# DavidSlayback/po-brax

Measured on AMD Instinct MI355X. Metric: env-steps/sec AntHeavenHell batch 65536 @1/2/4/8 GPU; % HBM roofline, higher is better.
Workload: dtype f32; 1 GPU; ant_heavenhell B=65536/GPU (global 65536), create(batch_size=B) autoreset chain, episode_length 1000, PBD 10 substeps, random uniform(-1,1) actions (threefry); env=ant_heavenhell, global_batch=65536, batch_per_gpu=65536, episode_length=1000, qp_storage=f32, parallelism=env-shard x1 (strong: global batch split), dynamics=pbd, obs_mask=none, obs_mask_columns=0, launch=hipGraph replay of the K steps

## Files before the change

po-brax_amd/csrc/pob_blockwalk.h:

```cpp
#pragma once
#include <stdint.h>
#ifdef POB_BW_HOST
#define POB_BW_D static inline
#else
#define POB_BW_D __device__ __forceinline__
#endif

#define QBW_WAVES 4
#define QBW_WCAP 50
#define QBW_SLOT_DW 11
#define QBW_CON_DW 5
#define QBW_LANE_MAX 64
#define QBW_CAP (QBW_WAVES * QBW_WCAP)
#define QBW_SEG_FLOATS (QBW_WCAP * QBW_SLOT_DW + 1)
#define QBW_NO_CONTACT (-1)

POB_BW_D constexpr int bw_item_off(const int j) { return QBW_SLOT_DW * j; }
POB_BW_D constexpr int bw_meta_off(const int j) { return QBW_SLOT_DW * j + 2 * QBW_CON_DW; }
POB_BW_D constexpr int bw_con_off(const int c) { return QBW_SLOT_DW * (c >> 1) + QBW_CON_DW * (c & 1); }
POB_BW_D constexpr int bw_count_off() { return QBW_WCAP * QBW_SLOT_DW; }

POB_BW_D constexpr int bw_meta(const int bit, const bool seg, const int slot) { return bit | (seg ? 64 : 0) | (slot << 7); }
POB_BW_D constexpr int bw_meta_bit(const int m) { return m & 63; }
POB_BW_D constexpr bool bw_meta_seg(const int m) { return (m & 64) != 0; }
POB_BW_D constexpr int bw_meta_slot(const int m) { return (m >> 7) & 3; }

POB_BW_D int bw_lane_count(const uint64_t m0, const uint64_t m1, const uint64_t m2) {
  const int n = __builtin_popcountll(m0) + __builtin_popcountll(m1) + __builtin_popcountll(m2);
  return n < QBW_LANE_MAX ? n : QBW_LANE_MAX;
}
POB_BW_D void bw_prefix_step(const uint64_t m, const int lane, const int b, int &base, int &tot) {
  base += __builtin_popcountll(m & ((1ull << lane) - 1ull)) << b;
  tot += __builtin_popcountll(m) << b;
}
#define QBW_PREFIX_BITS 7

POB_BW_D bool bw_next_item(uint64_t (&M)[3], int &slot, int &bit) {
  const bool h0 = M[0] != 0ull, h1 = M[1] != 0ull, h2 = M[2] != 0ull;
  const bool has = h0 | h1 | h2;
  slot = h0 ? 0 : (h1 ? 1 : 2);
  const uint64_t ml = h0 ? M[0] : (h1 ? M[1] : M[2]);
  bit = has ? __builtin_ctzll(ml) : 0;
  const uint64_t pop = has ? ml & (0ull - ml) : 0ull;
  M[0] = h0 ? M[0] & ~pop : M[0];
  M[1] = (!h0 & h1) ? M[1] & ~pop : M[1];
  M[2] = (!h0 & !h1) ? M[2] & ~pop : M[2];
  return has;
}

struct BwDeal {
  int off[QBW_WAVES];
  int T;
  bool ovf;
};
POB_BW_D BwDeal bw_deal(const int n0, const int n1, const int n2, const int n3, const int cap) {
  BwDeal d;
  d.off[0] = 0; d.off[1] = n0; d.off[2] = n0 + n1; d.off[3] = n0 + n1 + n2;
  const int T = n0 + n1 + n2 + n3;
  d.ovf = (T > cap) | (n0 > QBW_WCAP) | (n1 > QBW_WCAP) | (n2 > QBW_WCAP) | (n3 > QBW_WCAP);
  d.T = d.ovf ? 0 : T;
  return d;
}
POB_BW_D int bw_rounds(const BwDeal &d) { return (d.T + 7) >> 3; }
POB_BW_D int bw_first_round(const int w, const int sub) { return (w + sub) & (QBW_WAVES - 1); }
POB_BW_D void bw_item_owner(const BwDeal &d, const int i, int &w, int &j) {
  w = (i >= d.off[1] ? 1 : 0) + (i >= d.off[2] ? 1 : 0) + (i >= d.off[3] ? 1 : 0);
  j = i - (w == 0 ? 0 : (w == 1 ? d.off[1] : (w == 2 ? d.off[2] : d.off[3])));
}
POB_BW_D void bw_apply_range(const int base, const int n, const bool ovf, int &c0, int &c1) {
  c0 = 2 * base;
  c1 = ovf ? c0 : 2 * (base + n);
}
POB_BW_D void bw_body_ranges(const int base, const int n0, const int n1, const int n2, const bool ovf, int (&c)[4]) {
  c[0] = 2 * base;
  c[1] = ovf ? c[0] : c[0] + 2 * n0;
  c[2] = ovf ? c[0] : c[1] + 2 * n1;
  c[3] = ovf ? c[0] : c[2] + 2 * n2;
}
```

po-brax_amd/csrc/pob_kernels.hip:

```cpp
#include <hip/hip_fp16.h>
#include <hip/hip_runtime.h>

#include <climits>
#include <cstdio>
#include <cstdlib>
#include <cstring>
#include <mutex>
#include <new>
#include <type_traits>
#include <vector>

#include "../../include/pob.h"

#ifndef POB_QUAD_PRIO
#define POB_QUAD_PRIO 1
#endif
#ifndef POB_OCT_PRIO
#define POB_OCT_PRIO 1
#endif
#ifndef POB_HEX_PRIO
#define POB_HEX_PRIO 1
#endif
#include "pob_quad.h"
#include "pob_octet.h"
#include "pob_hexa.h"
#include "pob_physics.h"

namespace pob {
void default_params(pob_params &p);
const char *build_system(int kind, const pob_params &p, pob_sys &s);
int gather_grid(const pob_params &p, float *xyz, int cap);
}

struct pob_env {
  pob_sys sys;
  pob_sys *d_sys = nullptr;
  pob_params params;
  float *d_grid = nullptr;
  uint32_t *d_scratch = nullptr;
  int device = 0;
  int n_cu = 256;
};

#define POB_MIXED (-1)
#define POB_F_STAGED (1u << 16)
#define POB_F_INT_FORCE_FIXUP (1u << 30)
#define POB_F_INT_BWCAP_SHIFT 20
#define POB_F_INT_BWCAP_MASK (0xFFu << POB_F_INT_BWCAP_SHIFT)
#define POB_F_INTERNAL (POB_F_STAGED | POB_F_INT_FORCE_FIXUP | POB_F_INT_BWCAP_MASK)
#define POB_F_PUBLIC (POB_F_EPISODE | POB_F_AUTORESET | POB_F_ZERO_STEPS_ON_DONE)

#define POB_STATE_FIELDS(X)                                                                    \
  X(pos) X(rot) X(vel) X(ang) X(obs) X(reward) X(done) X(steps) X(truncation) X(m0) X(m1) X(m2) \
  X(rng) X(first_pos) X(first_rot) X(first_vel) X(first_ang) X(first_obs) X(any_done) X(done_u8) X(trunc_i32) \
  X(m0_i32) X(m1_i32) X(any_done_clear) X(obs_masked) X(ovf_mark)

struct StatePtrs {
  float *pos, *rot, *vel, *ang, *obs, *reward, *done, *steps, *truncation, *m0, *m1, *m2;
  uint32_t *rng;
  float *first_pos, *first_rot, *first_vel, *first_ang, *first_obs;
  uint32_t *any_done;
  uint8_t *done_u8;
  int32_t *trunc_i32, *m0_i32, *m1_i32;
  uint32_t *any_done_clear;
  float *obs_masked;
  uint8_t *ovf_mark;
};
POB_D void store_obs_masked(csys_t &S, float *dst, const float *stg, const int rows, const int D, const int lane) {
  const int K = S.obs_mask_n;
  for (int r = 0; r < rows; ++r)
    for (int c = lane; c < K; c += 64) dst[(size_t)r * K + c] = stg[r * D + S.obs_mask[c]];
}
static StatePtrs to_ptrs(const pob_state &s) {
  StatePtrs p;
#define POB_CP(f) p.f = s.f;
  POB_STATE_FIELDS(POB_CP)
#undef POB_CP
  return p;
}

template <typename QT> struct Q;
template <> struct Q<float> {
  static POB_D float ld(const float *p, size_t i) { return p[i]; }
  static POB_D void st(float *p, size_t i, float v) { p[i] = v; }
};
template <> struct Q<__half> {
  static POB_D float ld(const float *p, size_t i) { return __half2float(reinterpret_cast<const __half *>(p)[i]); }
  static POB_D void st(float *p, size_t i, float v) {
    asm volatile("" : "+v"(v));
    reinterpret_cast<__half *>(p)[i] = __float2half_rn(v);
  }
};
template <typename QT> POB_D v3 ld3(const float *p, size_t i) {
  return V(Q<QT>::ld(p, i), Q<QT>::ld(p, i + 1), Q<QT>::ld(p, i + 2));
}
template <typename QT> POB_D void st3(float *p, size_t i, v3 v) {
  Q<QT>::st(p, i, v.x); Q<QT>::st(p, i + 1, v.y); Q<QT>::st(p, i + 2, v.z);
}
template <typename QT> POB_D q4 ld4(const float *p, size_t i) {
  q4 q; q.w = Q<QT>::ld(p, i); q.x = Q<QT>::ld(p, i + 1); q.y = Q<QT>::ld(p, i + 2); q.z = Q<QT>::ld(p, i + 3);
  return q;
}
// ... 677 lines not shown
#endif
    constexpr int KBIT = KIND < 0 ? 16 : 1 << KIND;
    constexpr bool FASTP = (POB_QUAD_FAST_PASS & KBIT) != 0, REDER = (POB_QUAD_REDERIVE & KBIT) != 0;
    if (LEG) {
#pragma nounroll
      for (int it = 0; it < Sp->substeps; ++it) qlegacy_substep<KIND != POB_ANT>(Sp, LT, WT, bd, a, Ls);
    } else {
#if defined(POB_EXP_NO_COLLIDE)
#pragma nounroll
    for (int it = 0; it < 2 * iters; ++it) qpbd_substep<KIND != POB_ANT>(Sp, LT, WT, bd, a, Ls, false, S.friction);
#elif defined(POB_EXP_NO_PHYSICS)
#pragma nounroll
    for (int it = 0; it < 0 * iters; ++it) qpbd_substep<KIND != POB_ANT>(Sp, LT, WT, bd, a, Ls, false, S.friction);
#else
    constexpr bool TWO = KIND == POB_GATHER && POB_QUAD_TWO_PASS;
    constexpr bool WALLS = KIND != POB_ANT;
    int pass = TWO ? (__any(qwall_mask_margin(S, bd, POB_QUAD_NEAR_MARGIN) != 0u) ? 1 : 0) : 1;
    auto reload = [&]() {
#pragma unroll
      for (int l = 0; l < QNB; ++l) {
        const int g = qbody_global(l, k);
        bd.x[l] = ld3<QT>(in.pos, r3 + 3 * g);
        bd.q[l] = ld4<QT>(in.rot, r4 + 4 * g);
        bd.v[l] = ld3<QT>(in.vel, r3 + 3 * g);
        bd.w[l] = ld3<QT>(in.ang, r3 + 3 * g);
        Ls.set3(l, QF_CV, V(0.0f, 0.0f, 0.0f));
        Ls.set3(l, QF_CA, V(0.0f, 0.0f, 0.0f));
      }
    };
    for (;;) {
    if (pass == 0) {
      bool near = false;
#pragma nounroll
      for (int it = 0; it < 2 * iters; ++it) {
#if POB_QUAD_PRIO == 1
        const int lvl = (it * 4) / (2 * iters);
        if (lvl == 0) __builtin_amdgcn_s_setprio(3);
        else if (lvl == 1) __builtin_amdgcn_s_setprio(2);
        else if (lvl == 2) __builtin_amdgcn_s_setprio(1);
        else __builtin_amdgcn_s_setprio(0);
#endif
        qpbd_substep<false, true>(Sp, LT, WT, bd, a, Ls, (it & 1) != 0, fric, &near);
      }
      if (!__any(near)) break;
      pass = 1;
      reload();
      continue;
    }
#ifndef POB_QUAD_SLOW_OOL
#define POB_QUAD_SLOW_OOL 1
#endif
    if constexpr (MODE == 1 && WALLS && COOP) {
      const int capf = (int)((flags & POB_F_INT_BWCAP_MASK) >> POB_F_INT_BWCAP_SHIFT);
      QBlock blk{lds + QPOOL_OFF, __builtin_amdgcn_readfirstlane((int)threadIdx.x >> 6), 0,
                 capf != 0 ? capf : QBW_CAP, dead, false};
#pragma nounroll
      for (int it = 0; it < 2 * iters; ++it) {
#if POB_QUAD_PRIO == 1
        const int lvl = (it * 4) / (2 * iters);
        if (lvl == 0) __builtin_amdgcn_s_setprio(3);
        else if (lvl == 1) __builtin_amdgcn_s_setprio(2);
        else if (lvl == 2) __builtin_amdgcn_s_setprio(1);
        else __builtin_amdgcn_s_setprio(0);
#endif
        qpbd_substep<WALLS, false, false, true>(Sp, LT, WT, bd, a, Ls, (it & 1) != 0, fric, nullptr, nullptr, &blk);
      }
      if (dead) return;
      if (blk.ovf || (flags & POB_F_INT_FORCE_FIXUP)) {
        if (lane == 0) out.ovf_mark[b_first] = 1;
        return;
      }
      break;
    }
    if (MODE == 1 && WALLS) {
      bool ovf = false;
#pragma nounroll
      for (int it = 0; it < 2 * iters; ++it) {
#if POB_QUAD_PRIO == 1
        const int lvl = (it * 4) / (2 * iters);
        if (lvl == 0) __builtin_amdgcn_s_setprio(3);
        else if (lvl == 1) __builtin_amdgcn_s_setprio(2);
        else if (lvl == 2) __builtin_amdgcn_s_setprio(1);
        else __builtin_amdgcn_s_setprio(0);
#endif
        qpbd_substep<WALLS, false, false>(Sp, LT, WT, bd, a, Ls, (it & 1) != 0, fric, nullptr, &ovf);
        if (__any(ovf)) break;
      }
      if (__any(ovf) || (flags & POB_F_INT_FORCE_FIXUP)) {
        if (lane == 0) out.ovf_mark[b_first] = 1;
        return;
      }
      break;
    }
    if (pass == 1 && WALLS && FASTP && MODE == 0) {
      bool ovf = false;
#pragma nounroll
      for (int it = 0; it < 2 * iters; ++it) {
#if POB_QUAD_PRIO == 1
        const int lvl = (it * 4) / (2 * iters);
        if (lvl == 0) __builtin_amdgcn_s_setprio(3);
        else if (lvl == 1) __builtin_amdgcn_s_setprio(2);
        else if (lvl == 2) __builtin_amdgcn_s_setprio(1);
        else __builtin_amdgcn_s_setprio(0);
#endif
        qpbd_substep<WALLS, false, false>(Sp, LT, WT, bd, a, Ls, (it & 1) != 0, fric, nullptr, &ovf);
        if (__any(ovf)) break;
      }
      if (!__any(ovf)) break;
// ... 1631 lines not shown
    }
  }
  switch (kind) {
    case POB_HEAVENHELL: hipLaunchKernelGGL((k_step_hex<POB_HEAVENHELL, QT, GACC>), g, b, 0, st, sp, B, pi, act, po, flags, L); break;
    case POB_GATHER: hipLaunchKernelGGL((k_step_hex<POB_GATHER, QT, GACC>), g, b, 0, st, sp, B, pi, act, po, flags, L); break;
    case POB_TAG: hipLaunchKernelGGL((k_step_hex<POB_TAG, QT, GACC>), g, b, 0, st, sp, B, pi, act, po, flags, L); break;
    default: hipLaunchKernelGGL((k_step_hex<POB_ANT, QT, GACC>), g, b, 0, st, sp, B, pi, act, po, flags, L); break;
  }
}
template <typename QT>
static void launch_step_hex(int kind, int n_cu, hipStream_t st, const void *sp, int B, const StatePtrs &pi,
                            const float *act, const StatePtrs &po, uint32_t flags, int L) {
  const char *f = getenv("POB_HEX_GACC");
  const bool acc = f ? atoi(f) != 0 : (kind == POB_HEAVENHELL || kind == POB_TAG || (B + 3) / 4 <= 4 * n_cu);
  if (acc) launch_step_hex_g<QT, true>(kind, st, sp, B, pi, act, po, flags, L, n_cu);
  else launch_step_hex_g<QT, false>(kind, st, sp, B, pi, act, po, flags, L, n_cu);
}
template <typename QT, bool GACC>
static void launch_step_oct_g(int kind, hipStream_t st, const void *sp, int B, const StatePtrs &pi, const float *act,
                              const StatePtrs &po, uint32_t flags, int L) {
  const dim3 g((unsigned)((B + 7) / 8)), b(64);
  switch (kind) {
    case POB_HEAVENHELL: hipLaunchKernelGGL((k_step_oct<POB_HEAVENHELL, QT, GACC>), g, b, 0, st, sp, B, pi, act, po, flags, L); break;
    case POB_GATHER: hipLaunchKernelGGL((k_step_oct<POB_GATHER, QT, GACC>), g, b, 0, st, sp, B, pi, act, po, flags, L); break;
    case POB_TAG: hipLaunchKernelGGL((k_step_oct<POB_TAG, QT, GACC>), g, b, 0, st, sp, B, pi, act, po, flags, L); break;
    default: hipLaunchKernelGGL((k_step_oct<POB_ANT, QT, GACC>), g, b, 0, st, sp, B, pi, act, po, flags, L); break;
  }
}
template <typename QT>
static void launch_step_oct(int kind, int n_cu, hipStream_t st, const void *sp, int B, const StatePtrs &pi,
                            const float *act, const StatePtrs &po, uint32_t flags, int L) {
  const char *f = getenv("POB_OCT_GACC");
  const bool acc = f ? atoi(f) != 0 : (B + 7) / 8 <= 4 * n_cu;
  if (acc) launch_step_oct_g<QT, true>(kind, st, sp, B, pi, act, po, flags, L);
  else launch_step_oct_g<QT, false>(kind, st, sp, B, pi, act, po, flags, L);
}
#ifndef POB_QUAD_SPLIT_KINDS
#define POB_QUAD_SPLIT_KINDS 23
#endif
static bool quad_split_launch(int kind) {
  const char *f = getenv("POB_QUAD_SPLIT");
  if (f) return atoi(f) != 0;
  return ((POB_QUAD_SPLIT_KINDS >> (kind < 0 ? 4 : kind)) & 1) != 0;
}
static uint32_t quad_force_fixup() {
  const char *f = getenv("POB_QUAD_FORCE_FIXUP");
  return f && atoi(f) != 0 ? POB_F_INT_FORCE_FIXUP : 0u;
}
static uint32_t quad_block_cap() {
  const char *f = getenv("POB_QUAD_BLOCK_CAP");
  const int n = f ? atoi(f) : 0;
  return n >= 1 && n < QBW_CAP ? (uint32_t)n << POB_F_INT_BWCAP_SHIFT : 0u;
}
template <typename QT>
static void launch_step_quad(int kind, bool legacy, int n_cu, hipStream_t st, const void *sp, int B,
                             const StatePtrs &pi, const float *act, const StatePtrs &po, uint32_t flags, int L) {
  const int bs = 4 * B <= 64 * 256 ? 64 : 256;
  const dim3 g = grid_for(4 * B, bs), b(bs);
  if (legacy) {
    switch (kind) {
      case POB_HEAVENHELL: hipLaunchKernelGGL((k_step_legacy<POB_HEAVENHELL, QT>), g, b, 0, st, sp, B, pi, act, po, flags, L); break;
      case POB_GATHER: hipLaunchKernelGGL((k_step_legacy<POB_GATHER, QT>), g, b, 0, st, sp, B, pi, act, po, flags, L); break;
      case POB_TAG: hipLaunchKernelGGL((k_step_legacy<POB_TAG, QT>), g, b, 0, st, sp, B, pi, act, po, flags, L); break;
      default: hipLaunchKernelGGL((k_step_legacy<POB_ANT, QT>), g, b, 0, st, sp, B, pi, act, po, flags, L); break;
    }
    return;
  }
  if (kind == POB_GATHER && (size_t)4 * B <= (size_t)3 * 64 * 4 * n_cu) {
    hipLaunchKernelGGL((k_step_quad_ga3<QT>), g, b, 0, st, sp, B, pi, act, po, flags, L);
    return;
  }
  const bool split = quad_split_launch(kind) && po.ovf_mark != nullptr;
  flags |= split ? quad_force_fixup() : 0u;
  const bool coop = split && bs == 256 && (kind == POB_HEAVENHELL || kind == POB_TAG);
  flags |= coop ? quad_block_cap() : 0u;
  switch (kind) {
    case POB_HEAVENHELL:
      if (split) {
        if (coop) hipLaunchKernelGGL((k_step_quad<POB_HEAVENHELL, QT, 1, true>), g, b, 0, st, sp, B, pi, act, po, flags, L);
        else hipLaunchKernelGGL((k_step_quad<POB_HEAVENHELL, QT, 1>), g, b, 0, st, sp, B, pi, act, po, flags, L);
        hipLaunchKernelGGL((k_step_quad<POB_HEAVENHELL, QT, 2>), g, b, 0, st, sp, B, pi, act, po, flags, L);
      } else {
        hipLaunchKernelGGL((k_step_quad<POB_HEAVENHELL, QT>), g, b, 0, st, sp, B, pi, act, po, flags, L);
      }
      break;
    case POB_GATHER:
      if (split) {
        hipLaunchKernelGGL((k_step_quad<POB_GATHER, QT, 1>), g, b, 0, st, sp, B, pi, act, po, flags, L);
        hipLaunchKernelGGL((k_step_quad<POB_GATHER, QT, 2>), g, b, 0, st, sp, B, pi, act, po, flags, L);
      } else {
        hipLaunchKernelGGL((k_step_quad<POB_GATHER, QT>), g, b, 0, st, sp, B, pi, act, po, flags, L);
      }
      break;
    case POB_TAG:
      if (split) {
        if (coop) hipLaunchKernelGGL((k_step_quad<POB_TAG, QT, 1, true>), g, b, 0, st, sp, B, pi, act, po, flags, L);
        else hipLaunchKernelGGL((k_step_quad<POB_TAG, QT, 1>), g, b, 0, st, sp, B, pi, act, po, flags, L);
        hipLaunchKernelGGL((k_step_quad<POB_TAG, QT, 2>), g, b, 0, st, sp, B, pi, act, po, flags, L);
      } else {
        hipLaunchKernelGGL((k_step_quad<POB_TAG, QT>), g, b, 0, st, sp, B, pi, act, po, flags, L);
      }
      break;
    default: hipLaunchKernelGGL((k_step_quad<POB_ANT, QT>), g, b, 0, st, sp, B, pi, act, po, flags, L); break;
  }
}
extern "C" {

int pob_abi_version(void) { return POB_ABI_VERSION; }
const char *pob_last_error(void) { return g_err; }

int pob_default_params(pob_params *p) {
  if (!p) return fail(POB_EINVAL, "params is NULL");
  pob::default_params(*p);
  return POB_OK;
}

static std::mutex g_grave_mu;
static std::vector<void *> g_grave;

static void drain_grave() {
  std::vector<void *> dead;
  {
    std::lock_guard<std::mutex> lk(g_grave_mu);
    dead.swap(g_grave);
  }
  for (void *p : dead) (void)hipFree(p);
}

// ... 295 lines not shown
```

po-brax_amd/csrc/pob_quad.h:

```cpp
#pragma once
#include "pob_physics.h"

#define QNB 3
#define QNJ 2

struct QBody {
  v3 x[QNB];
  q4 q[QNB];
  v3 v[QNB];
  v3 w[QNB];
};

template <int J>
POB_D float quad_bcast(float x) {
  float r;
  if (J == 0)
    asm volatile("s_nop 1\n\tv_mov_b32_dpp %0, %1 quad_perm:[0,0,0,0] row_mask:0xf bank_mask:0xf" : "=&v"(r) : "v"(x));
  else if (J == 1)
    asm volatile("s_nop 1\n\tv_mov_b32_dpp %0, %1 quad_perm:[1,1,1,1] row_mask:0xf bank_mask:0xf" : "=&v"(r) : "v"(x));
  else if (J == 2)
    asm volatile("s_nop 1\n\tv_mov_b32_dpp %0, %1 quad_perm:[2,2,2,2] row_mask:0xf bank_mask:0xf" : "=&v"(r) : "v"(x));
  else
    asm volatile("s_nop 1\n\tv_mov_b32_dpp %0, %1 quad_perm:[3,3,3,3] row_mask:0xf bank_mask:0xf" : "=&v"(r) : "v"(x));
  return r;
// ... 47 lines not shown
  }
  POB_D static constexpr int torso_off(int f) {
    return f == QF_PX ? QLT_PX : (f == QF_PQ ? QLT_PQ : (f == QF_CV ? QLT_CV : QLT_CA));
  }
  POB_D float *at(int l, int f, int i) const {
    return l == 0 ? base + 64 * QLL_FLOATS + 16 * (torso_off(f) + i) + (t >> 2) : base + 64 * (lane_off(l, f) + i) + t;
  }
  POB_D v3 get3(int l, int f) const { return V(*at(l, f, 0), *at(l, f, 1), *at(l, f, 2)); }
  POB_D q4 get4(int l, int f) const {
    q4 q; q.w = *at(l, f, 0); q.x = *at(l, f, 1); q.y = *at(l, f, 2); q.z = *at(l, f, 3); return q;
  }
  POB_D void set3(int l, int f, v3 v) const {
    if (l != 0 || (t & 3) == 0) { *at(l, f, 0) = v.x; *at(l, f, 1) = v.y; *at(l, f, 2) = v.z; }
  }
  POB_D void set4(int l, int f, q4 q) const {
    if (l != 0 || (t & 3) == 0) { *at(l, f, 0) = q.w; *at(l, f, 1) = q.x; *at(l, f, 2) = q.y; *at(l, f, 3) = q.z; }
  }
  POB_D v3 get3_lane(int l, int f, int lane) const {
    const float *p = base + 64 * lane_off(l, f) + lane;
    return V(p[0], p[64], p[128]);
  }
  POB_D float *head() const { return base + 64 * QLL_HEAD + t; }
  POB_D float *pool() const { return base + QPOOL_OFF; }
};

POB_D constexpr int qcontact_body(int c) { return c == 0 ? 0 : (c == 1 ? 2 : c - 2); }

POB_D v3 qcap_end(csys_t &S, const float *LT, int l, int q) {
  if (l == 0) return SV(S.cap_end[0][q]);
  const float *e = LT + POB_LEG_BODY(l) + 2 + 3 * q;
  return V(e[0], e[1], e[2]);
}
POB_D v3 qground_end(csys_t &S, const float *LT, int c) {
  if (c == 0) return SV(S.ground_end[0]);
  return V(LT[POB_LEG_GROUND], LT[POB_LEG_GROUND + 1], LT[POB_LEG_GROUND + 2]);
}
POB_D float qground_r(csys_t &S, const float *LT, int c) {
  return c == 0 ? S.ground_r[0] : LT[POB_LEG_GROUND + 3];
}

struct QGround {
  float pen[2];
};
struct QMesh {
  v3 a[QNB], b[QNB];
};
#ifndef QK
#define QK 12
#endif
struct QWalls {
  int nct;
  float c[6 * QK];
  float seg[6 * QNB];
  int cb[QNB + 1];
};
#ifndef POB_QUAD_WAVE_WALK
#define POB_QUAD_WAVE_WALK 1
#endif
#if POB_QUAD_WAVE_WALK
#define QWALK mesh_wave_walk
#else
#define QWALK mesh_lane_walk
#endif

POB_D void qground_detect(csys_t &S, const float *LT, const QBody &b, const v3 rv_leg, QGround &gc, v3 (&pe)[2]) {
  pe[0] = S.torso_point ? b.x[0] : vadd(b.x[0], qrot(qground_end(S, LT, 0), b.q[0]));
  pe[1] = vsub(b.x[2], rv_leg);
  gc.pen[0] = qground_r(S, LT, 0) - pe[0].z;
  gc.pen[1] = qground_r(S, LT, 1) - pe[1].z;
}

POB_D uint32_t qwall_mask(csys_t &S, const QBody &b) {
  float mnx = b.x[0].x, mxx = b.x[0].x, mny = b.x[0].y, mxy = b.x[0].y;
#pragma unroll
  for (int l = 1; l < QNB; ++l) {
    mnx = fminf(mnx, b.x[l].x); mxx = fmaxf(mxx, b.x[l].x);
    mny = fminf(mny, b.x[l].y); mxy = fmaxf(mxy, b.x[l].y);
  }
#ifdef POB_EXP_NO_WALLS
  const int nw = 0;
#else
  const int nw = S.n_walls;
#endif
  uint32_t m = 0u;
#pragma unroll
  for (int w = 0; w < POB_MAXW; ++w) {
    const float lx = S.wall_lo[w][0], ly = S.wall_lo[w][1], hx = S.wall_hi[w][0], hy = S.wall_hi[w][1];
    const bool near = (mnx <= hx) & (mxx >= lx) & (mny <= hy) & (mxy >= ly);
    m |= (near & (w < nw)) ? 1u << w : 0u;
  }
  return m;
}

POB_D uint32_t qwall_mask_margin(csys_t &S, const QBody &b, const float margin) {
  float mnx = b.x[0].x, mxx = b.x[0].x, mny = b.x[0].y, mxy = b.x[0].y;
#pragma unroll
  for (int l = 1; l < QNB; ++l) {
    mnx = fminf(mnx, b.x[l].x); mxx = fmaxf(mxx, b.x[l].x);
    mny = fminf(mny, b.x[l].y); mxy = fmaxf(mxy, b.x[l].y);
  }
  const int nw = S.n_walls;
  uint32_t m = 0u;
#pragma unroll
  for (int w = 0; w < POB_MAXW; ++w) {
    const float lx = S.wall_lo[w][0] - margin, ly = S.wall_lo[w][1] - margin;
    const float hx = S.wall_hi[w][0] + margin, hy = S.wall_hi[w][1] + margin;
    const bool near = (mnx <= hx) & (mxx >= lx) & (mny <= hy) & (mxy >= ly);
    m |= (near & (w < nw)) ? 1u << w : 0u;
// ... 187 lines not shown
    QMesh ms;
    qmesh_segments(S, LT, b, rv_leg, ms);
    const uint32_t lw = qwall_mask(S, b);
    qmesh_items(S, LT, WT, lw | (lw << 8) | (lw << 16), ms, M);
  }
#ifdef POB_EXP_NO_WALK
  return;
#endif
#ifdef POB_EXP_WALK_DEAD
  if (S.n_walls < 64) return;
#endif
#ifdef POB_EXP_CULL_ONLY
  {
    uint32_t k0 = (uint32_t)M[0], k1 = (uint32_t)M[1], k2 = (uint32_t)M[2];
    asm volatile("" : "+v"(k0), "+v"(k1), "+v"(k2));
    int z = (int)((k0 ^ k1 ^ k2) & 0u);
    asm volatile("" : "+v"(z));
    ws.nct = z;
    return;
  }
#endif
  if (!__any((M[0] | M[1] | M[2]) != 0ull)) return;
#if POB_QUAD_WAVE_WALK
  if (!OVF) {
    qwalls_walk_pool(S, LT, WT, b, M, ws, L, *ovf);
    return;
  }
  qwalls_walk<false>(S, LT, WT, b, M, ws);
#else
  ws.nct = qwalls_walk_ool(Sp, LT, WT, b.x[0], b.x[1], b.x[2], b.q[0], b.q[1], b.q[2], M[0], M[1], M[2], &ws);
#endif
#ifdef POB_EXP_NO_APPLY
  {
    int z = ws.nct & 0;
    asm volatile("" : "+v"(z));
    ws.nct = z;
  }
#endif
  if (!OVF) {
    *ovf = *ovf | (ws.nct > QK);
    return;
  }
  if (ws.nct > QK) {
    QMesh ms;
    qmesh_segments(S, LT, b, rv_leg, ms);
#pragma unroll
    for (int l = 0; l < QNB; ++l) {
      ws.seg[6 * l] = ms.a[l].x; ws.seg[6 * l + 1] = ms.a[l].y; ws.seg[6 * l + 2] = ms.a[l].z;
      ws.seg[6 * l + 3] = ms.b[l].x; ws.seg[6 * l + 4] = ms.b[l].y; ws.seg[6 * l + 5] = ms.b[l].z;
    }
  }
}

struct QBlock {
  float *xch;
  int w;
  int sub;
  int cap;
  bool dead;
  bool ovf;
};
static_assert(QBW_SEG_FLOATS <= QL_FLOATS * 64 - QPOOL_OFF, "a wave's exchange segment fits its former contact pool");
POB_D void qblock_barrier() { asm volatile("s_waitcnt lgkmcnt(0)\n\ts_barrier" ::: "memory"); }

POB_D void qwalls_detect_block(csys_t *Sp, const float *LT, const float *WT, const QBody &b, QWalls &ws, const QLds &L,
                               QBlock &blk) {
  csys_t &S = *launder(Sp);
  uint64_t M[QNB];
  QMesh ms;
  {
    const v3 rv_leg = qrot_xy(qcap_end(S, LT, 2, 0), b.q[2]);
    qmesh_segments(S, LT, b, rv_leg, ms);
    const uint32_t lw = qwall_mask(S, b);
    qmesh_items(S, LT, WT, lw | (lw << 8) | (lw << 16), ms, M);
  }
  if (blk.dead) { M[0] = 0ull; M[1] = 0ull; M[2] = 0ull; }
#ifdef POB_EXP_NO_WALK
  M[0] = 0ull; M[1] = 0ull; M[2] = 0ull;
#endif
  float *own = L.pool();
  const int nl = bw_lane_count(M[0], M[1], M[2]);
  int nb[QNB];
#pragma unroll
  for (int l = 0; l < QNB; ++l) nb[l] = __builtin_popcountll(M[l]);
  int base = 0, tot = 0;
#pragma unroll
  for (int bit = 0; bit < QBW_PREFIX_BITS; ++bit) bw_prefix_step(__ballot(((nl >> bit) & 1) != 0), L.t, bit, base, tot);
  {
    int at = base;
#pragma unroll
    for (int l = 0; l < QNB; ++l) {
      const float r = q_cap_r(S, LT, l);
      uint64_t m = M[l];
#pragma nounroll
      while (__any(m != 0ull)) {
        const bool has = m != 0ull;
        const int bit = has ? __builtin_ctzll(m) : 0;
        m &= m - 1ull;
        if (has && at < QBW_WCAP) {
          float *o = own + bw_item_off(at);
          const float meta = __int_as_float(bw_meta(bit, l != 0, l));
          o[0] = ms.a[l].x; o[1] = ms.a[l].y; o[2] = ms.a[l].z; o[3] = ms.b[l].x; o[4] = ms.b[l].y; o[5] = ms.b[l].z;
          o[6] = r; o[7] = meta;
          o[2 * QBW_CON_DW] = meta;
        }
        at += has ? 1 : 0;
      }
    }
  }
  if (L.t == 0) own[bw_count_off()] = __int_as_float(tot);
  qblock_barrier();
  const int ws_f = QL_FLOATS * 64;
  const int n0 = __builtin_amdgcn_readfirstlane(__float_as_int(blk.xch[bw_count_off()]));
  const int n1 = __builtin_amdgcn_readfirstlane(__float_as_int(blk.xch[ws_f + bw_count_off()]));
  const int n2 = __builtin_amdgcn_readfirstlane(__float_as_int(blk.xch[2 * ws_f + bw_count_off()]));
  const int n3 = __builtin_amdgcn_readfirstlane(__float_as_int(blk.xch[3 * ws_f + bw_count_off()]));
  const BwDeal d = bw_deal(n0, n1, n2, n3, blk.cap);
  blk.ovf = blk.ovf | d.ovf;
  {
    GuardBranch g;
    mesh_block_walk(g, WT, pob_face_table(S), S.wall_cz, S.wall_hz, blk.xch, ws_f, d, bw_first_round(blk.w, blk.sub));
  }
  qblock_barrier();
  ++blk.sub;
  bw_body_ranges(base, nb[0], nb[1], nb[2], d.ovf, ws.cb);
#ifdef POB_EXP_NO_APPLY
  {
    int z = ws.cb[0];
    asm volatile("" : "+v"(z));
    ws.cb[1] = z; ws.cb[2] = z; ws.cb[3] = z;
  }
#endif
  ws.nct = ws.cb[QNB] - ws.cb[0];
}

POB_D int qblock_next_hit(const float *sg, int c, const int c1) {
#pragma unroll 1
  while (true) {
    const bool skip = c < c1 && __float_as_int(sg[bw_con_off(c) + QBW_CON_DW - 1]) == QBW_NO_CONTACT;
    if (!__any(skip)) break;
    c = skip ? c + 1 : c;
  }
  return c;
}

template <class G>
POB_D void qwall_pos_one(G &g, csys_t &S, const HCon &SC, const float *LT, const v3 (&x)[QNB], const q4 (&q)[QNB],
                         const v3 (&px)[QNB], const q4 (&pq)[QNB], const int l, const float tau, const v3 n,
                         const float dist, v3 (&DX)[QNB], v3 (&DA)[QNB]) {
  const v3 xl = qpick3(l, x);
  const q4 ql = qpick4(l, q);
  const v3 pe = l == 0 ? xl : qseg_point(LT, l, xl, ql, tau);
  v3 dx = qpick3(l, DX), da = qpick3(l, DA);
  owall_position(g, SC, q_cap_r(S, LT, l) - dist, pe, n, 1e-6f + dist, q_inv_mass(S, LT, l), xl, ql, qpick4(l, pq),
                 qpick3(l, px), dx, da);
  qput3(l, DX, dx);
  qput3(l, DA, da);
}
template <class G>
POB_D void qwall_vel_one(G &g, csys_t &S, const HCon &SC, const float *LT, const v3 (&x)[QNB], const q4 (&q)[QNB],
                         const v3 (&v)[QNB], const v3 (&w)[QNB], const int l, const float tau, const v3 n,
                         const float dist, v3 (&dV)[QNB], v3 (&dW)[QNB]) {
  const v3 xl = qpick3(l, x);
  const v3 pe = l == 0 ? xl : qseg_point(LT, l, xl, qpick4(l, q), tau);
  v3 dv = qpick3(l, dV), dw = qpick3(l, dW);
  ocontact_vel_pe(g, SC, false, q_cap_r(S, LT, l) - dist, pe, n, 1e-6f + dist, q_inv_mass(S, LT, l), xl, qpick3(l, v),
                  qpick3(l, w), dv, dw);
  qput3(l, dV, dv);
  qput3(l, dW, dw);
}

struct QOvf {
  v3 x[QNB], px[QNB], v[QNB], w[QNB], a[QNB], b[QNB], d0[QNB], d1[QNB];
  q4 q[QNB], pq[QNB];
  float fric;
  int on;
};
template <bool VEL>
__device__ __attribute__((noinline)) void qwalls_rewalk(csys_t *Sp, const float *LT, const float *WT, QOvf *st) {
  csys_t &S = *launder(Sp);
  GuardBranch g;
  const HCon SC{st->fric, S.inv_h};
  v3 x[QNB], px[QNB], v[QNB], w[QNB], d0[QNB], d1[QNB];
  q4 q[QNB], pq[QNB];
  QMesh ms;
#pragma unroll
// ... 21 lines not shown
POB_D void qwalls_rewalk_inl(csys_t &S, const float *LT, const float *WT, const QBody &b, const QLds &L,
                             const QWalls &ws, const bool ovf, const float fric, v3 (&d0)[QNB], v3 (&d1)[QNB]) {
  GuardBranch g;
  const HCon SC{fric, S.inv_h};
  QMesh ms;
#pragma unroll
  for (int l = 0; l < QNB; ++l) {
    ms.a[l] = V(ws.seg[6 * l], ws.seg[6 * l + 1], ws.seg[6 * l + 2]);
    ms.b[l] = V(ws.seg[6 * l + 3], ws.seg[6 * l + 4], ws.seg[6 * l + 5]);
  }
  const uint32_t wa = ovf ? (1u << S.n_walls) - 1u : 0u;
  uint64_t M[QNB];
  qmesh_items(S, LT, WT, wa | (wa << 8) | (wa << 16), ms, M);
  mesh_wave_walk<QNB, false>(g, WT, pob_face_table(S), S.wall_cz, S.wall_hz, M,
             [&](const int l, v3 &A, v3 &B, float &r, bool &seg) { qmesh_seg(S, LT, ms, l, A, B, r, seg); },
             [&](const int l, const int, const float tau, const v3 n, const float dist) {
    if constexpr (VEL) {
      qwall_vel_one(g, S, SC, LT, b.x, b.q, b.v, b.w, l, tau, n, dist, d0, d1);
    } else {
      v3 px[QNB];
      q4 pq[QNB];
#pragma unroll
      for (int k = 0; k < QNB; ++k) { px[k] = L.get3(k, QF_PX); pq[k] = L.get4(k, QF_PQ); }
      qwall_pos_one(g, S, SC, LT, b.x, b.q, px, pq, l, tau, n, dist, d0, d1);
    }
  });
}

template <bool WALLS, bool OVF = true, bool COOP = false>
POB_D void qcontacts_position(csys_t *Sp, const float *LT, const float *WT, QBody &b, const QLds &L, QGround &gc,
                              const QWalls &ws, v3 (&DX)[QNB], v3 (&DA)[QNB], const float fric) {
  csys_t &S = *launder(Sp);
  const HCon SC{fric, S.inv_h};
  GuardBranch g;
  {
    const v3 rv_leg = qrot_xy(qcap_end(S, LT, 2, 0), b.q[2]);
    v3 pe[2];
    qground_detect(S, LT, b, rv_leg, gc, pe);
#pragma unroll
    for (int c = 0; c < 2; ++c) {
      POB_FENCE();
      const int l = qcontact_body(c);
      if (gc.pen[c] > 0.0f)
        oground_position(g, SC, gc.pen[c], pe[c], qground_r(S, LT, c), q_inv_mass(S, LT, l), b.x[l], b.q[l],
                         L.get4(l, QF_PQ), L.get3(l, QF_PX), DX[l], DA[l]);
    }
  }
  if (!WALLS || !__any(ws.nct != 0)) return;
  POB_FENCE();
  if constexpr (COOP) {
    const float *sg = L.pool();
#pragma unroll
    for (int l = 0; l < QNB; ++l) {
      const int c1 = ws.cb[l + 1];
      if (!__any(ws.cb[l] < c1)) continue;
      const v3 px = L.get3(l, QF_PX);
      const q4 pq = L.get4(l, QF_PQ);
      const v3 rv = l == 0 ? V(0.0f, 0.0f, 0.0f) : qrot_xy(qcap_end(S, LT, l, 0), b.q[l]);
      const float r = q_cap_r(S, LT, l), im = q_inv_mass(S, LT, l);
      int c = qblock_next_hit(sg, ws.cb[l], c1);
#pragma unroll 1
      while (__any(c < c1)) {
        if (c < c1) {
          const float *p = sg + bw_con_off(c);
          const float tau = p[0], dist = p[4];
          const v3 pe = l == 0 ? b.x[0] : vfma(rv, tau, b.x[l]);
          owall_position(g, SC, r - dist, pe, V(p[1], p[2], p[3]), 1e-6f + dist, im, b.x[l], b.q[l], pq, px, DX[l], DA[l]);
          ++c;
        }
        c = qblock_next_hit(sg, c, c1);
      }
    }
    return;
  }
  v3 px[QNB];
  q4 pq[QNB];
#pragma unroll
  for (int l = 0; l < QNB; ++l) { px[l] = L.get3(l, QF_PX); pq[l] = L.get4(l, QF_PQ); }
#if POB_QUAD_WAVE_WALK
  if (!OVF) {
    const float *pool = L.pool();
    int ci = ws.nct > 0 ? __float_as_int(*L.head()) : -1;
#pragma unroll 1
    while (__any(ci >= 0)) {
      if (ci >= 0) {
        const float *c = pool + 6 * ci;
        const int meta = __float_as_int(c[5]);
        qwall_pos_one(g, S, SC, LT, b.x, b.q, px, pq, meta & 3, c[0], V(c[1], c[2], c[3]), c[4], DX, DA);
        ci = (meta >> 2) - 1;
      }
    }
    return;
  }
#endif
  const bool ovf = ws.nct > QK;
  const int nc = ovf ? 0 : ws.nct;
#pragma unroll 1
  for (int i = 0; i < QK; ++i) {
    if (!__any(i < nc)) break;
    if (i < nc) {
      const float *c = ws.c + 6 * i;
      qwall_pos_one(g, S, SC, LT, b.x, b.q, px, pq, (int)c[0], c[1], V(c[2], c[3], c[4]), c[5], DX, DA);
    }
  }
  if (!OVF) return;
#if POB_QUAD_REWALK_INLINE
#ifndef POB_EXP_NO_REWALK
  if (__any(ovf)) qwalls_rewalk_inl<false>(S, LT, WT, b, L, ws, ovf, fric, DX, DA);
#endif
  if (false) {
#else
  if (__any(ovf)) {
#endif
    QOvf st;
#pragma unroll
    for (int l = 0; l < QNB; ++l) {
      st.x[l] = b.x[l]; st.q[l] = b.q[l]; st.px[l] = px[l]; st.pq[l] = pq[l]; st.d0[l] = DX[l]; st.d1[l] = DA[l];
      st.a[l] = V(ws.seg[6 * l], ws.seg[6 * l + 1], ws.seg[6 * l + 2]);
      st.b[l] = V(ws.seg[6 * l + 3], ws.seg[6 * l + 4], ws.seg[6 * l + 5]);
    }
    st.fric = fric;
    st.on = ovf ? 1 : 0;
    qwalls_rewalk<false>(Sp, LT, WT, &st);
#pragma unroll
    for (int l = 0; l < QNB; ++l) { DX[l] = st.d0[l]; DA[l] = st.d1[l]; b.x[l] = st.x[l]; b.q[l] = st.q[l]; }
  }
}

template <bool WALLS, bool OVF = true, bool COOP = false>
POB_D void qcontacts_velocity(csys_t *Sp, const float *LT, const float *WT, QBody &b, const QGround &gc,
                              const QWalls &ws, const QLds &L, v3 (&dV)[QNB], v3 (&dW)[QNB], const float fric) {
  csys_t &S = *launder(Sp);
  const HCon SC{fric, S.inv_h};
  GuardBranch g;
#pragma unroll
  for (int c = 0; c < 2; ++c) {
    POB_FENCE();
    const int l = qcontact_body(c);
    if (gc.pen[c] > 0.0f) {
      const v3 e = qground_end(S, LT, c);
      const v3 pe = l == 0 ? vadd(b.x[0], qrot(e, b.q[0])) : vadd(b.x[l], qrot_xy(e, b.q[l]));
      ocontact_vel_pe(g, SC, true, gc.pen[c], pe, V(0.0f, 0.0f, 1.0f), qground_r(S, LT, c), q_inv_mass(S, LT, l), b.x[l],
                      b.v[l], b.w[l], dV[l], dW[l]);
    }
  }
  if (!WALLS || !__any(ws.nct != 0)) return;
#ifdef POB_EXP_NO_VWALK
  return;
#endif
  POB_FENCE();
  if constexpr (COOP) {
    const float *sg = L.pool();
#pragma unroll
    for (int l = 0; l < QNB; ++l) {
      const int c1 = ws.cb[l + 1];
      if (!__any(ws.cb[l] < c1)) continue;
      const v3 rv = l == 0 ? V(0.0f, 0.0f, 0.0f) : qrot_xy(qcap_end(S, LT, l, 0), b.q[l]);
      const float r = q_cap_r(S, LT, l), im = q_inv_mass(S, LT, l);
      int c = qblock_next_hit(sg, ws.cb[l], c1);
#pragma unroll 1
      while (__any(c < c1)) {
        if (c < c1) {
          const float *p = sg + bw_con_off(c);
          const float tau = p[0], dist = p[4];
          const v3 pe = l == 0 ? b.x[0] : vfma(rv, tau, b.x[l]);
          ocontact_vel_pe(g, SC, false, r - dist, pe, V(p[1], p[2], p[3]), 1e-6f + dist, im, b.x[l], b.v[l], b.w[l], dV[l],
                          dW[l]);
          ++c;
        }
        c = qblock_next_hit(sg, c, c1);
      }
    }
    return;
  }
#if POB_QUAD_WAVE_WALK
  if (!OVF) {
    const float *pool = L.pool();
    int ci = ws.nct > 0 ? __float_as_int(*L.head()) : -1;
#pragma unroll 1
    while (__any(ci >= 0)) {
      if (ci >= 0) {
        const float *c = pool + 6 * ci;
        const int meta = __float_as_int(c[5]);
        qwall_vel_one(g, S, SC, LT, b.x, b.q, b.v, b.w, meta & 3, c[0], V(c[1], c[2], c[3]), c[4], dV, dW);
        ci = (meta >> 2) - 1;
      }
    }
    return;
  }
#endif
  const bool ovf = ws.nct > QK;
  const int nc = ovf ? 0 : ws.nct;
#pragma unroll 1
  for (int i = 0; i < QK; ++i) {
    if (!__any(i < nc)) break;
    if (i < nc) {
      const float *c = ws.c + 6 * i;
      qwall_vel_one(g, S, SC, LT, b.x, b.q, b.v, b.w, (int)c[0], c[1], V(c[2], c[3], c[4]), c[5], dV, dW);
    }
  }
  if (!OVF) return;
#if POB_QUAD_REWALK_INLINE
#ifndef POB_EXP_NO_REWALK
  if (__any(ovf)) qwalls_rewalk_inl<true>(S, LT, WT, b, QLds{nullptr, 0}, ws, ovf, fric, dV, dW);
#endif
  if (false) {
#else
  if (__any(ovf)) {
#endif
    QOvf st;
#pragma unroll
    for (int l = 0; l < QNB; ++l) {
      st.x[l] = b.x[l]; st.q[l] = b.q[l]; st.v[l] = b.v[l]; st.w[l] = b.w[l]; st.d0[l] = dV[l]; st.d1[l] = dW[l];
      st.a[l] = V(ws.seg[6 * l], ws.seg[6 * l + 1], ws.seg[6 * l + 2]);
      st.b[l] = V(ws.seg[6 * l + 3], ws.seg[6 * l + 4], ws.seg[6 * l + 5]);
    }
    st.fric = fric;
    st.on = ovf ? 1 : 0;
    qwalls_rewalk<true>(Sp, LT, WT, &st);
#pragma unroll
    for (int l = 0; l < QNB; ++l) {
      dV[l] = st.d0[l]; dW[l] = st.d1[l];
      b.x[l] = st.x[l]; b.q[l] = st.q[l]; b.v[l] = st.v[l]; b.w[l] = st.w[l];
    }
// ... 332 lines not shown
```

Measured before the change: 501.1 million env-steps/s.

## Dedupe torso wall items per quad and precompute per-body hit bitmasks

```diff
diff --git a/po-brax_amd/csrc/pob_blockwalk.h b/po-brax_amd/csrc/pob_blockwalk.h
--- a/po-brax_amd/csrc/pob_blockwalk.h
+++ b/po-brax_amd/csrc/pob_blockwalk.h
@@ -34,6 +34,8 @@
   tot += __builtin_popcountll(m) << b;
 }
 #define QBW_PREFIX_BITS 7
+#define QBW_PREFIX_SHORT_BITS 2
+POB_BW_D constexpr bool bw_prefix_needs_all(const int count) { return count >= (1 << QBW_PREFIX_SHORT_BITS); }
 
 POB_BW_D bool bw_next_item(uint64_t (&M)[3], int &slot, int &bit) {
   const bool h0 = M[0] != 0ull, h1 = M[1] != 0ull, h2 = M[2] != 0ull;
@@ -77,3 +79,20 @@
   c[2] = ovf ? c[0] : c[1] + 2 * n1;
   c[3] = ovf ? c[0] : c[2] + 2 * n2;
 }
+
+POB_BW_D constexpr bool bw_quad_lead(const int lane) { return (lane & 3) == 0; }
+POB_BW_D constexpr int bw_quad_torso_count(const int lane, const int n0) { return bw_quad_lead(lane) ? n0 : 0; }
+POB_BW_D void bw_quad_ranges(const int lane, const int base0, const int n0, const int base, const int n1, const int n2,
+                             const bool ovf, int (&c)[5]) {
+  c[0] = 2 * base0;
+  c[1] = ovf ? c[0] : c[0] + 2 * n0;
+  c[2] = 2 * (base + bw_quad_torso_count(lane, n0));
+  c[3] = ovf ? c[2] : c[2] + 2 * n1;
+  c[4] = ovf ? c[2] : c[3] + 2 * n2;
+}
+
+#define QBW_HIT_ITEMS 16
+POB_BW_D constexpr uint32_t bw_hit_bits(const bool h0, const bool h1, const int i) {
+  return ((h0 ? 1u : 0u) | (h1 ? 2u : 0u)) << (2 * i);
+}
+POB_BW_D constexpr int bw_hit_count(const int tot, const bool wide) { return wide && tot <= QBW_WCAP ? QBW_WCAP + 1 : tot; }
diff --git a/po-brax_amd/csrc/pob_kernels.hip b/po-brax_amd/csrc/pob_kernels.hip
--- a/po-brax_amd/csrc/pob_kernels.hip
+++ b/po-brax_amd/csrc/pob_kernels.hip
@@ -47,7 +47,9 @@
 #define POB_F_INT_FORCE_FIXUP (1u << 30)
 #define POB_F_INT_BWCAP_SHIFT 20
 #define POB_F_INT_BWCAP_MASK (0xFFu << POB_F_INT_BWCAP_SHIFT)
-#define POB_F_INTERNAL (POB_F_STAGED | POB_F_INT_FORCE_FIXUP | POB_F_INT_BWCAP_MASK)
+#define POB_F_INT_HITW_SHIFT 17
+#define POB_F_INT_HITW_MASK (0x7u << POB_F_INT_HITW_SHIFT)
+#define POB_F_INTERNAL (POB_F_STAGED | POB_F_INT_FORCE_FIXUP | POB_F_INT_BWCAP_MASK | POB_F_INT_HITW_MASK)
 #define POB_F_PUBLIC (POB_F_EPISODE | POB_F_AUTORESET | POB_F_ZERO_STEPS_ON_DONE)
 
 #define POB_STATE_FIELDS(X)                                                                    \
@@ -831,8 +833,9 @@
 #endif
     if constexpr (MODE == 1 && WALLS && COOP) {
       const int capf = (int)((flags & POB_F_INT_BWCAP_MASK) >> POB_F_INT_BWCAP_SHIFT);
+      const int hitf = (int)((flags & POB_F_INT_HITW_MASK) >> POB_F_INT_HITW_SHIFT);
       QBlock blk{lds + QPOOL_OFF, __builtin_amdgcn_readfirstlane((int)threadIdx.x >> 6), 0,
-                 capf != 0 ? capf : QBW_CAP, dead, false};
+                 capf != 0 ? capf : QBW_CAP, hitf != 0 ? hitf : QBW_HIT_ITEMS, dead, false};
 #pragma nounroll
       for (int it = 0; it < 2 * iters; ++it) {
 #if POB_QUAD_PRIO == 1
@@ -2570,6 +2573,11 @@
   const int n = f ? atoi(f) : 0;
   return n >= 1 && n < QBW_CAP ? (uint32_t)n << POB_F_INT_BWCAP_SHIFT : 0u;
 }
+static uint32_t quad_hit_width() {
+  const char *f = getenv("POB_QUAD_HIT_WIDTH");
+  const int n = f ? atoi(f) : 0;
+  return n >= 1 && n <= 7 ? (uint32_t)n << POB_F_INT_HITW_SHIFT : 0u;
+}
 template <typename QT>
 static void launch_step_quad(int kind, bool legacy, int n_cu, hipStream_t st, const void *sp, int B,
                              const StatePtrs &pi, const float *act, const StatePtrs &po, uint32_t flags, int L) {
@@ -2591,7 +2599,7 @@
   const bool split = quad_split_launch(kind) && po.ovf_mark != nullptr;
   flags |= split ? quad_force_fixup() : 0u;
   const bool coop = split && bs == 256 && (kind == POB_HEAVENHELL || kind == POB_TAG);
-  flags |= coop ? quad_block_cap() : 0u;
+  flags |= coop ? quad_block_cap() | quad_hit_width() : 0u;
   switch (kind) {
     case POB_HEAVENHELL:
       if (split) {
diff --git a/po-brax_amd/csrc/pob_quad.h b/po-brax_amd/csrc/pob_quad.h
--- a/po-brax_amd/csrc/pob_quad.h
+++ b/po-brax_amd/csrc/pob_quad.h
@@ -123,8 +123,10 @@
   int nct;
   float c[6 * QK];
   float seg[6 * QNB];
-  int cb[QNB + 1];
+  int cb[QNB + 2];
+  uint32_t hm[QNB];
 };
+POB_D constexpr int qcb_lo(const int l) { return l == 0 ? 0 : l + 1; }
 #ifndef POB_QUAD_WAVE_WALK
 #define POB_QUAD_WAVE_WALK 1
 #endif
@@ -418,11 +420,21 @@
   }
 }
 
+#ifndef POB_QUAD_TORSO_ONCE
+#define POB_QUAD_TORSO_ONCE 1
+#endif
+#ifndef POB_QUAD_HIT_MASK
+#define POB_QUAD_HIT_MASK 1
+#endif
+#ifndef POB_QUAD_PREFIX_SHORT
+#define POB_QUAD_PREFIX_SHORT 1
+#endif
 struct QBlock {
   float *xch;
   int w;
   int sub;
   int cap;
+  int hitw;
   bool dead;
   bool ovf;
 };
@@ -445,13 +457,35 @@
   M[0] = 0ull; M[1] = 0ull; M[2] = 0ull;
 #endif
   float *own = L.pool();
+#if POB_QUAD_TORSO_ONCE
+  {
+    const uint32_t lo = (uint32_t)__float_as_int(quad_bcast<0>(__int_as_float((int)(uint32_t)M[0])));
+    const uint32_t hi = (uint32_t)__float_as_int(quad_bcast<0>(__int_as_float((int)(uint32_t)(M[0] >> 32))));
+    M[0] = ((uint64_t)hi << 32) | lo;
+  }
+  const int n0 = __builtin_popcountll(M[0]);
+  if (!bw_quad_lead(L.t)) M[0] = 0ull;
+#else
+  const int n0 = __builtin_popcountll(M[0]);
+#endif
+  const int n1 = __builtin_popcountll(M[1]), n2 = __builtin_popcountll(M[2]);
   const int nl = bw_lane_count(M[0], M[1], M[2]);
-  int nb[QNB];
-#pragma unroll
-  for (int l = 0; l < QNB; ++l) nb[l] = __builtin_popcountll(M[l]);
   int base = 0, tot = 0;
+#if POB_QUAD_PREFIX_SHORT
+#pragma unroll
+  for (int bit = 0; bit < QBW_PREFIX_SHORT_BITS; ++bit) bw_prefix_step(__ballot(((nl >> bit) & 1) != 0), L.t, bit, base, tot);
+  if (__any(bw_prefix_needs_all(nl))) {
+#pragma unroll
+    for (int bit = QBW_PREFIX_SHORT_BITS; bit < QBW_PREFIX_BITS; ++bit)
+      bw_prefix_step(__ballot(((nl >> bit) & 1) != 0), L.t, bit, base, tot);
+  }
+#else
 #pragma unroll
   for (int bit = 0; bit < QBW_PREFIX_BITS; ++bit) bw_prefix_step(__ballot(((nl >> bit) & 1) != 0), L.t, bit, base, tot);
+#endif
+#if POB_QUAD_HIT_MASK
+  tot = bw_hit_count(tot, __any((n0 > blk.hitw) | (n1 > blk.hitw) | (n2 > blk.hitw)) != 0);
+#endif
   {
     int at = base;
 #pragma unroll
@@ -477,11 +511,11 @@
   if (L.t == 0) own[bw_count_off()] = __int_as_float(tot);
   qblock_barrier();
   const int ws_f = QL_FLOATS * 64;
-  const int n0 = __builtin_amdgcn_readfirstlane(__float_as_int(blk.xch[bw_count_off()]));
-  const int n1 = __builtin_amdgcn_readfirstlane(__float_as_int(blk.xch[ws_f + bw_count_off()]));
-  const int n2 = __builtin_amdgcn_readfirstlane(__float_as_int(blk.xch[2 * ws_f + bw_count_off()]));
-  const int n3 = __builtin_amdgcn_readfirstlane(__float_as_int(blk.xch[3 * ws_f + bw_count_off()]));
-  const BwDeal d = bw_deal(n0, n1, n2, n3, blk.cap);
+  const int w0 = __builtin_amdgcn_readfirstlane(__float_as_int(blk.xch[bw_count_off()]));
+  const int w1 = __builtin_amdgcn_readfirstlane(__float_as_int(blk.xch[ws_f + bw_count_off()]));
+  const int w2 = __builtin_amdgcn_readfirstlane(__float_as_int(blk.xch[2 * ws_f + bw_count_off()]));
+  const int w3 = __builtin_amdgcn_readfirstlane(__float_as_int(blk.xch[3 * ws_f + bw_count_off()]));
+  const BwDeal d = bw_deal(w0, w1, w2, w3, blk.cap);
   blk.ovf = blk.ovf | d.ovf;
   {
     GuardBranch g;
@@ -489,15 +523,41 @@
   }
   qblock_barrier();
   ++blk.sub;
-  bw_body_ranges(base, nb[0], nb[1], nb[2], d.ovf, ws.cb);
+#if POB_QUAD_TORSO_ONCE
+  const int base0 = __float_as_int(quad_bcast<0>(__int_as_float(base)));
+  bw_quad_ranges(L.t, base0, n0, base, n1, n2, d.ovf, ws.cb);
+#else
+  {
+    int c[QNB + 1];
+    bw_body_ranges(base, n0, n1, n2, d.ovf, c);
+    ws.cb[0] = c[0]; ws.cb[1] = c[1]; ws.cb[2] = c[1]; ws.cb[3] = c[2]; ws.cb[4] = c[3];
+  }
+#endif
 #ifdef POB_EXP_NO_APPLY
   {
-    int z = ws.cb[0];
-    asm volatile("" : "+v"(z));
-    ws.cb[1] = z; ws.cb[2] = z; ws.cb[3] = z;
-  }
-#endif
-  ws.nct = ws.cb[QNB] - ws.cb[0];
+    int z = ws.cb[0], y = ws.cb[2];
+    asm volatile("" : "+v"(z), "+v"(y));
+    ws.cb[1] = z; ws.cb[3] = y; ws.cb[4] = y;
+  }
+#endif
+  ws.nct = (ws.cb[1] - ws.cb[0]) + (ws.cb[4] - ws.cb[2]);
+#if POB_QUAD_HIT_MASK
+#pragma unroll
+  for (int l = 0; l < QNB; ++l) {
+    const int c0 = ws.cb[qcb_lo(l)], n = (ws.cb[qcb_lo(l) + 1] - c0) >> 1;
+    uint32_t hm = 0u;
+#pragma unroll 1
+    for (int i = 0; __any(i < n); ++i) {
+      if (i < n) {
+        const float *p = own + bw_con_off(c0 + 2 * i);
+        hm |= bw_hit_bits(__float_as_int(p[QBW_CON_DW - 1]) != QBW_NO_CONTACT,
+                          __float_as_int(p[2 * QBW_CON_DW - 1]) != QBW_NO_CONTACT, i);
+      }
+    }
+    ws.hm[l] = hm;
+  }
+  ws.nct = (int)(ws.hm[0] | ws.hm[1] | ws.hm[2]);
+#endif
 }
 
 POB_D int qblock_next_hit(const float *sg, int c, const int c1) {
@@ -625,24 +685,41 @@
     const float *sg = L.pool();
 #pragma unroll
     for (int l = 0; l < QNB; ++l) {
-      const int c1 = ws.cb[l + 1];
-      if (!__any(ws.cb[l] < c1)) continue;
+#if POB_QUAD_HIT_MASK
+      uint32_t hm = ws.hm[l];
+      if (!__any(hm != 0u)) continue;
+#else
+      const int c1 = ws.cb[qcb_lo(l) + 1];
+      if (!__any(ws.cb[qcb_lo(l)] < c1)) continue;
+#endif
       const v3 px = L.get3(l, QF_PX);
       const q4 pq = L.get4(l, QF_PQ);
       const v3 rv = l == 0 ? V(0.0f, 0.0f, 0.0f) : qrot_xy(qcap_end(S, LT, l, 0), b.q[l]);
       const float r = q_cap_r(S, LT, l), im = q_inv_mass(S, LT, l);
-      int c = qblock_next_hit(sg, ws.cb[l], c1);
+      const auto apply = [&](const float *p) {
+        const float tau = p[0], dist = p[4];
+        const v3 pe = l == 0 ? b.x[0] : vfma(rv, tau, b.x[l]);
+        owall_position(g, SC, r - dist, pe, V(p[1], p[2], p[3]), 1e-6f + dist, im, b.x[l], b.q[l], pq, px, DX[l], DA[l]);
+      };
+#if POB_QUAD_HIT_MASK
+#pragma unroll 1
+      while (__any(hm != 0u)) {
+        if (hm != 0u) {
+          apply(sg + bw_con_off(ws.cb[qcb_lo(l)] + __builtin_ctz(hm)));
+          hm &= hm - 1u;
+        }
+      }
+#else
+      int c = qblock_next_hit(sg, ws.cb[qcb_lo(l)], c1);
 #pragma unroll 1
       while (__any(c < c1)) {
         if (c < c1) {
-          const float *p = sg + bw_con_off(c);
-          const float tau = p[0], dist = p[4];
-          const v3 pe = l == 0 ? b.x[0] : vfma(rv, tau, b.x[l]);
-          owall_position(g, SC, r - dist, pe, V(p[1], p[2], p[3]), 1e-6f + dist, im, b.x[l], b.q[l], pq, px, DX[l], DA[l]);
+          apply(sg + bw_con_off(c));
           ++c;
         }
         c = qblock_next_hit(sg, c, c1);
       }
+#endif
     }
     return;
   }
@@ -726,23 +803,40 @@
     const float *sg = L.pool();
 #pragma unroll
     for (int l = 0; l < QNB; ++l) {
-      const int c1 = ws.cb[l + 1];
-      if (!__any(ws.cb[l] < c1)) continue;
+#if POB_QUAD_HIT_MASK
+      uint32_t hm = ws.hm[l];
+      if (!__any(hm != 0u)) continue;
+#else
+      const int c1 = ws.cb[qcb_lo(l) + 1];
+      if (!__any(ws.cb[qcb_lo(l)] < c1)) continue;
+#endif
       const v3 rv = l == 0 ? V(0.0f, 0.0f, 0.0f) : qrot_xy(qcap_end(S, LT, l, 0), b.q[l]);
       const float r = q_cap_r(S, LT, l), im = q_inv_mass(S, LT, l);
-      int c = qblock_next_hit(sg, ws.cb[l], c1);
+      const auto apply = [&](const float *p) {
+        const float tau = p[0], dist = p[4];
+        const v3 pe = l == 0 ? b.x[0] : vfma(rv, tau, b.x[l]);
+        ocontact_vel_pe(g, SC, false, r - dist, pe, V(p[1], p[2], p[3]), 1e-6f + dist, im, b.x[l], b.v[l], b.w[l], dV[l],
+                        dW[l]);
+      };
+#if POB_QUAD_HIT_MASK
+#pragma unroll 1
+      while (__any(hm != 0u)) {
+        if (hm != 0u) {
+          apply(sg + bw_con_off(ws.cb[qcb_lo(l)] + __builtin_ctz(hm)));
+          hm &= hm - 1u;
+        }
+      }
+#else
+      int c = qblock_next_hit(sg, ws.cb[qcb_lo(l)], c1);
 #pragma unroll 1
       while (__any(c < c1)) {
         if (c < c1) {
-          const float *p = sg + bw_con_off(c);
-          const float tau = p[0], dist = p[4];
-          const v3 pe = l == 0 ? b.x[0] : vfma(rv, tau, b.x[l]);
-          ocontact_vel_pe(g, SC, false, r - dist, pe, V(p[1], p[2], p[3]), 1e-6f + dist, im, b.x[l], b.v[l], b.w[l], dV[l],
-                          dW[l]);
+          apply(sg + bw_con_off(c));
           ++c;
         }
         c = qblock_next_hit(sg, c, c1);
       }
+#endif
     }
     return;
   }
```

Result: faster. 541.3 million env-steps/s, median of 6 (+8.0%).
